# ebeauce/Seismic_BPMF

Measured on AMD Instinct MI355X. Metric: million network-CC-samples/s (matched filter), higher is better.
Workload: dtype f32

## Files before the change

### seismic_bpmf_amd/csrc/mf_split.h

```cpp
#pragma once
#include <hip/hip_runtime.h>
#include <cstdint>

namespace bpmf {
namespace sp {

typedef _Float16 f16x8 __attribute__((ext_vector_type(8)));
typedef float f32x16 __attribute__((ext_vector_type(16)));
typedef float f32x4 __attribute__((ext_vector_type(4)));
typedef float f32x4u __attribute__((ext_vector_type(4), aligned(4)));
typedef int i32x4 __attribute__((ext_vector_type(4)));
typedef int i32x2 __attribute__((ext_vector_type(2)));
typedef unsigned u32x4 __attribute__((ext_vector_type(4)));

constexpr int NT = 2;
constexpr int LAGS_W = 1024 * NT;
constexpr int WAVES = 4;
constexpr int THREADS = 64 * WAVES;
constexpr int LAGS_WG = WAVES * LAGS_W;
constexpr int W_LOADS = 10;
constexpr int W_CHUNKS = 64 * W_LOADS;
constexpr int W_BYTES = (W_CHUNKS + W_CHUNKS / 8) * 16;
constexpr int B_LOADS = 4;
constexpr int BAND_BYTES = 64 * B_LOADS * 16;
constexpr int BAND_PLANE = BAND_BYTES / 2;
constexpr int WAVE_LDS = W_BYTES + BAND_BYTES;
constexpr int WG_LDS = WAVES * WAVE_LDS;
constexpr int MAX_KS = 26;
constexpr int BAND_LEAD = 40;
constexpr int S_TARGET = 14;
constexpr int S_CLAMP = 60;
constexpr float SP_MAX_NORM = 1000.0f;

__host__ __device__ inline int nks_of(int L) { return (L + 38 + 15) / 16; }
__host__ __device__ inline int max_segment_len() { return (16 * MAX_KS - 38) / 8 * 8; }
__host__ __device__ inline int n_segments_of(int L) { return (L + max_segment_len() - 1) / max_segment_len(); }
__host__ __device__ inline int segment_len_of(int L)
{
    const int n = n_segments_of(L);
    return ((L + n - 1) / n + 7) / 8 * 8;
}
__host__ __device__ inline int max_template_len() { return 4096; }
__host__ __device__ inline int band_e_dwords(int nks) { return 8 * nks + 32; }
__host__ __device__ inline int band_o_off(int nks)
{
    const int e = band_e_dwords(nks);
    return e + ((17 - e % 32) + 32) % 32;
}
__host__ __device__ inline size_t split_row_bytes(size_t N) { return ((N + 7) / 8) * 32; }

__host__ __device__ inline int scale_exp_of(unsigned maxbits)
{
    if (maxbits == 0u || maxbits >= 0x7f800000u) return 0;
    const int e = (int)(maxbits >> 23) - 127;
    int s = S_TARGET - e;
    if (s > S_CLAMP) s = S_CLAMP;
    if (s < -S_CLAMP) s = -S_CLAMP;
    return s;
}
__host__ __device__ inline float pow2f(int s)
{
    union { unsigned u; float f; } v;
    v.u = (unsigned)(s + 127) << 23;
    return v.f;
}

constexpr float LO_SCALE = 2048.0f;

__device__ __forceinline__ void split_one(float v, float lo_scale, unsigned short& hi, unsigned short& lo)
{
    const _Float16 h = (_Float16)v;
    const float res = v - (float)h;
    const _Float16 l = (_Float16)(res * lo_scale);
    hi = __builtin_bit_cast(unsigned short, h);
    lo = __builtin_bit_cast(unsigned short, l);
}

__global__ __launch_bounds__(256) void sp_absmax_kernel(const float* __restrict__ data, size_t N,
                                                        unsigned* __restrict__ maxbits)
{
    const float* d = data + (size_t)blockIdx.y * N;
    unsigned m = 0;
    for (size_t i = (size_t)blockIdx.x * 256 + threadIdx.x; i < N; i += (size_t)gridDim.x * 256)
        m = max(m, __float_as_uint(d[i]) & 0x7fffffffu);
#pragma unroll
    for (int o = 32; o > 0; o >>= 1) m = max(m, (unsigned)__shfl_xor((int)m, o));
    if ((threadIdx.x & 63) == 0 && m) atomicMax(maxbits + blockIdx.y, m);
}

__global__ void sp_scale_kernel(const unsigned* __restrict__ maxbits, int n_ch, int* __restrict__ s_exp,
                                float* __restrict__ scd)
{
    const int ch = blockIdx.x * blockDim.x + threadIdx.x;
    if (ch >= n_ch) return;
    const int s = scale_exp_of(maxbits[ch]);
    s_exp[ch] = s;
    scd[ch] = pow2f(-s);
}

__global__ __launch_bounds__(256) void sp_split_data_kernel(const float* __restrict__ data, size_t N, size_t NQ,
                                                            const int* __restrict__ s_exp, u32x4* __restrict__ out)
{
    const size_t q = (size_t)blockIdx.x * 256 + threadIdx.x;
    if (q >= NQ) return;
    const size_t ch = blockIdx.y;
    const float* d = data + ch * N + 8 * q;
    const float sc = pow2f(s_exp[ch]);
    float v[8];
    if (8 * q + 8 <= N) {
        const f32x4u a = *(const f32x4u*)d, b = *(const f32x4u*)(d + 4);
#pragma unroll
        for (int i = 0; i < 4; ++i) { v[i] = a[i]; v[4 + i] = b[i]; }
    } else {
#pragma unroll
        for (int i = 0; i < 8; ++i) v[i] = 8 * q + i < N ? d[i] : 0.0f;
    }
    unsigned short hi[8], lo[8];
#pragma unroll
    for (int i = 0; i < 8; ++i) split_one(v[i] * sc, LO_SCALE, hi[i], lo[i]);
    u32x4 oh, ol;
#pragma unroll
    for (int i = 0; i < 4; ++i) {
        oh[i] = (unsigned)hi[2 * i] | ((unsigned)hi[2 * i + 1] << 16);
        ol[i] = (unsigned)lo[2 * i] | ((unsigned)lo[2 * i + 1] << 16);
    }
    u32x4* o = out + (ch * NQ + q) * 2;
    o[0] = oh;
    o[1] = ol;
}

__global__ __launch_bounds__(64) void sp_band_kernel(const float* __restrict__ tmpl, const int* __restrict__ mv,
                                                     int L, int n_seg, int seg_len, unsigned* __restrict__ bands,
                                                     float* __restrict__ sct)
{
    const size_t tc = blockIdx.x / (unsigned)n_seg;
    const int seg = (int)(blockIdx.x % (unsigned)n_seg);
    const int lane = threadIdx.x;
    const float* x = tmpl + tc * (size_t)L;
    unsigned m = 0;
    for (int l = lane; l < L; l += 64) m = max(m, __float_as_uint(x[l]) & 0x7fffffffu);
#pragma unroll
    for (int o = 32; o > 0; o >>= 1) m = max(m, (unsigned)__shfl_xor((int)m, o));
    const int s = scale_exp_of(m);
    const float sc = pow2f(s);
    if (lane == 0 && seg == 0) sct[tc] = pow2f(-s);
    const int mvc = mv[tc];
    const int r = ((mvc % 8) + 8) % 8;
    const int nks = nks_of(seg_len);
    const int e_d = band_e_dwords(nks), o_off = band_o_off(nks);
    unsigned* img = bands + (size_t)blockIdx.x * (BAND_BYTES / 4);
    auto elem = [&](int i, int p) -> unsigned {
        const int ls = i - BAND_LEAD - r;
        const int l = seg * seg_len + ls;
        if (ls < 0 || ls >= seg_len || l >= L) return 0u;
        unsigned short hi, lo;
        split_one(x[l] * sc, 1.0f, hi, lo);
        return p ? lo : hi;
    };
    for (int w = lane; w < BAND_BYTES / 4; w += 64) {
        const int p = w >= BAND_PLANE / 4 ? 1 : 0;
        const int n = w - p * (BAND_PLANE / 4);
        unsigned val = 0u;
        if (n < e_d) val = elem(2 * n, p) | (elem(2 * n + 1, p) << 16);
        else if (n >= o_off && n < o_off + e_d) {
            const int k = n - o_off;
            val = elem(2 * k + 1, p) | (elem(2 * k + 2, p) << 16);
        }
        img[w] = val;
    }
}

__device__ __forceinline__ bool sp_tile_of_block(unsigned bid, int T, int n_lag_blocks, int& t, long long& lag_block)
{
    const unsigned xcd = bid & 7u, i = bid >> 3;
    const unsigned total = (unsigned)n_lag_blocks * (unsigned)T;
    const unsigned per_xcd = (total + 7u) >> 3;
    const unsigned flat = xcd * per_xcd + i;
    t = (int)(flat % (unsigned)T);
    lag_block = (long long)(flat / (unsigned)T);
    return i < per_xcd && flat < total;
}

#define SP_SB __builtin_amdgcn_sched_barrier(0)
#define SP_RD2(dst, addr, o0) \
    asm volatile("ds_read2_b32 %0, %1 offset0:%2 offset1:%3" : "=v"(dst) : "v"(addr), "n"(o0), "n"((o0) + 1))
#define SP_RD128(dst, addr, off) asm volatile("ds_read_b128 %0, %1 offset:%2" : "=v"(dst) : "v"(addr), "n"(off))

struct Frags {
    i32x2 a[2][2];
    i32x4 b[NT][2];
};

__device__ __forceinline__ f16x8 sp_h8(i32x2 lo, i32x2 hi)
{
    const i32x4 v = {lo[0], lo[1], hi[0], hi[1]};
    return __builtin_bit_cast(f16x8, v);
}
__device__ __forceinline__ f16x8 sp_h8(i32x4 v) { return __builtin_bit_cast(f16x8, v); }

template <bool NETWORK_SUM, bool STEP1, int ABLATE = 0, bool SEGMENTED = false>
__global__ __launch_bounds__(THREADS, 2) void mf_split_kernel(
    const u32x4* __restrict__ sdata, const unsigned* __restrict__ bands, const float* __restrict__ sct,
    const float* __restrict__ scd, const int4* __restrict__ chan_rec, const float* __restrict__ e_d,
    const int2* __restrict__ range, int L, long long N, int T, int n_ch, long long n_corr, int step,
    float* __restrict__ out, int n_lag_blocks, int lag_block0, int prio, int n_seg, int seg_len)
{
    extern __shared__ __attribute__((aligned(16))) char sp_smem[];
    const int tid = threadIdx.x;
    const int lane = tid & 63;
    const int wv = __builtin_amdgcn_readfirstlane(tid >> 6);
    const int a = lane & 31;
    const int g = lane >> 5;
    const int nks = nks_of(seg_len);
    const bool kprio = (((blockIdx.x >> 3) ^ (blockIdx.x >> 8)) & 1u) != 0;

    int t;
    long long lag_block;
    if (!sp_tile_of_block(blockIdx.x, T, n_lag_blocks, t, lag_block)) return;
    lag_block += lag_block0;
    const int2 rgi = range[t];
    const long long lag0 = lag_block * LAGS_WG + (long long)wv * LAGS_W;
    const int2 rg = make_int2(rgi.x * step, rgi.y * step);
    const long long nwin = N - L + 1;
    const size_t row_bytes = split_row_bytes((size_t)N);

    f32x16 sum[NT];
#pragma unroll
    for (int u = 0; u < NT; ++u)
#pragma unroll
        for (int r = 0; r < 16; ++r) sum[u][r] = 0.0f;

    const bool wave_valid = rg.x <= rg.y && !(lag0 > rg.y || lag0 + LAGS_W - 1 < rg.x);
    const bool wave_inside = lag0 >= rg.x && lag0 + LAGS_W - 1 <= rg.y;
    const long long lag_w = lag0 + 32 * a + 4 * g;

    if (wave_valid) {
        char* wbase = sp_smem + wv * WAVE_LDS;
        char* bbase = wbase + W_BYTES;
        const unsigned w_st = (unsigned)(size_t)wbase + 16u * (unsigned)(lane + (lane >> 3));
        const unsigned b_st = (unsigned)(size_t)bbase + 16u * (unsigned)lane;
        const unsigned b_rd = (unsigned)(size_t)wbase + 144u * (unsigned)a + 32u * (unsigned)g;
        const int odd = a & 1;
        const int a_dw = 4 * g - ((a + 1) >> 1) + BAND_LEAD / 2 + (odd ? band_o_off(nks) : 0);
        const unsigned a_rd = (unsigned)(size_t)bbase + 4u * (unsigned)a_dw;
        const int4* __restrict__ recs = chan_rec + (size_t)t * (n_ch + 2);

        u32x4 rd[W_LOADS], rt[B_LOADS];
        auto issue_stage = [&](int ch, int mvc, int sg) {
            const __amdgpu_buffer_rsrc_t rs = __builtin_amdgcn_make_buffer_rsrc(
                (void*)((const char*)sdata + (size_t)ch * row_bytes), 0, (int)row_bytes, 0x00020000);
            const long long q0 = (lag0 >> 3) + (long long)(mvc >> 3) + (long long)sg * (seg_len >> 3);
            const unsigned o = (unsigned)(q0 * 32 + 16 * lane);
            if (q0 >= 0) {
#pragma unroll
                for (int i = 0; i < W_LOADS; ++i)
                    rd[i] = __builtin_bit_cast(u32x4, __builtin_amdgcn_raw_buffer_load_b128(rs, (int)(o + 1024u * i), 0, 0));
            } else {
                unsigned oo = o;
#pragma unroll
                for (int i = 0; i < W_LOADS; ++i) {
                    asm volatile("" : "+v"(oo));
                    rd[i] = __builtin_bit_cast(u32x4, __builtin_amdgcn_raw_buffer_load_b128(rs, (int)oo, 0, 0));
                    oo += 1024u;
                }
            }
            const u32x4* bi = (const u32x4*)(bands + (((size_t)t * n_ch + ch) * n_seg + sg) * (BAND_BYTES / 4)) + lane;
#pragma unroll
            for (int i = 0; i < B_LOADS; ++i) rt[i] = bi[64 * i];
        };
        auto write_stage = [&]() {
#pragma unroll
            for (int i = 0; i < B_LOADS; ++i)
                asm volatile("ds_write_b128 %0, %1 offset:%2" :: "v"(b_st), "v"(rt[i]), "n"(1024 * i) : "memory");
#pragma unroll
            for (int i = 0; i < W_LOADS; ++i)
                asm volatile("ds_write_b128 %0, %1 offset:%2" :: "v"(w_st), "v"(rd[i]), "n"(1152 * i) : "memory");
        };

        int4 rec = recs[0];
        int4 rec1 = recs[1];
        int ri = 0, seg = 0;
        f32x16 acc[NT];
        f32x4 ed[NT][4];
        if (ABLATE < 2 && rec.x >= 0) issue_stage(rec.x, rec.y, 0);
        while (rec.x >= 0) {
            const int ch = rec.x;
            const bool last_seg = !SEGMENTED || seg == n_seg - 1;
            if constexpr (ABLATE < 2) write_stage();
            const float w = __int_as_float(rec.z);
            const int mvc = rec.y;
            const float rt_n = __int_as_float(rec.w);
            const float s_t = sct[(size_t)t * n_ch + ch];
            const float s_d = scd[ch];
            const float s_td = s_t * s_d;
            const int4 rec2 = recs[ri + 2];
            const float* edc = e_d + (size_t)ch * (size_t)nwin;
            if (!last_seg) {
            } else if constexpr (ABLATE >= 1) {
#pragma unroll
                for (int u = 0; u < NT; ++u)
#pragma unroll
                    for (int i = 0; i < 4; ++i) ed[u][i] = (f32x4){1.0f, 1.0f, 1.0f, 1.0f};
            } else if (wave_inside) {
#pragma unroll
                for (int u = 0; u < NT; ++u)
#pragma unroll
                    for (int i = 0; i < 4; ++i) ed[u][i] = *(const f32x4u*)(edc + lag_w + 1024 * u + 8 * i + mvc);
            } else {
#pragma unroll
                for (int u = 0; u < NT; ++u)
#pragma unroll
                    for (int i = 0; i < 4; ++i) {
                        const long long lag = lag_w + 1024 * u + 8 * i;
                        if (lag + 3 >= rg.x && lag <= rg.y) ed[u][i] = *(const f32x4u*)(edc + lag + mvc);
                        else ed[u][i] = (f32x4){0.0f, 0.0f, 0.0f, 0.0f};
                    }
            }
            if constexpr (ABLATE < 2) {
                if (!last_seg) issue_stage(rec.x, rec.y, seg + 1);
                else if (rec1.x >= 0) issue_stage(rec1.x, rec1.y, 0);
            }

            if (!SEGMENTED || seg == 0) {
#pragma unroll
                for (int u = 0; u < NT; ++u)
#pragma unroll
                    for (int r = 0; r < 16; ++r) acc[u][r] = 0.0f;
            }

            unsigned ap = a_rd, ap2 = a_rd + BAND_PLANE, bp = b_rd;
            Frags f[2];
#define SP_REQ(s, dw, off)                                                    \
    SP_RD2(f[s].a[0][0], ap, (dw));     SP_RD2(f[s].a[0][1], ap, (dw) + 2);   \
    SP_RD128(f[s].b[0][0], bp, (off));         SP_RD128(f[s].b[1][0], bp, (off) + 4608);      \
    SP_RD128(f[s].b[0][1], bp, (off) + 16);    SP_RD128(f[s].b[1][1], bp, (off) + 4608 + 16); \
    SP_RD2(f[s].a[1][0], ap2, (dw));    SP_RD2(f[s].a[1][1], ap2, (dw) + 2)
#define SP_MFMA(acc, av, bv) acc = __builtin_amdgcn_mfma_f32_32x32x16_f16(av, bv, acc, 0, 0, 0)
#define SP_WAIT(n) asm volatile("s_waitcnt lgkmcnt(%0)" :: "n"(n) : "memory")
#define SP_STEP(cur, nxt, dw, off)                                                          \
    {                                                                                        \
        SP_WAIT(5); SP_SB;                                                                   \
        const f16x8 ah = sp_h8(f[cur].a[0][0], f[cur].a[0][1]);                              \
        const f16x8 hs = ah * (_Float16)(1.0f / LO_SCALE);       \
        SP_MFMA(acc[0], ah, sp_h8(f[cur].b[0][0]));                                          \
        SP_SB;                                                                               \
        SP_RD2(f[nxt].a[0][0], ap, (dw)); SP_RD2(f[nxt].a[0][1], ap, (dw) + 2);              \
        SP_WAIT(6); SP_SB;                                                                   \
        SP_MFMA(acc[1], ah, sp_h8(f[cur].b[1][0]));                                          \
        SP_SB;                                                                               \
        SP_RD128(f[nxt].b[0][0], bp, (off)); SP_RD128(f[nxt].b[1][0], bp, (off) + 4608);     \
        SP_WAIT(7); SP_SB;                                                                   \
        SP_MFMA(acc[0], hs, sp_h8(f[cur].b[0][1]));                                          \
        SP_SB;                                                                               \
        SP_RD128(f[nxt].b[0][1], bp, (off) + 16); SP_RD128(f[nxt].b[1][1], bp, (off) + 4608 + 16); \
        SP_WAIT(8); SP_SB;                                                                   \
        SP_MFMA(acc[1], hs, sp_h8(f[cur].b[1][1]));                                          \
        SP_SB;                                                                               \
        SP_RD2(f[nxt].a[1][0], ap2, (dw)); SP_RD2(f[nxt].a[1][1], ap2, (dw) + 2);            \
        SP_WAIT(8); SP_SB;                                                                   \
        const f16x8 al = sp_h8(f[cur].a[1][0], f[cur].a[1][1]);                              \
        SP_MFMA(acc[0], al, sp_h8(f[cur].b[0][0]));                                          \
        SP_SB;                                                                               \
        SP_MFMA(acc[1], al, sp_h8(f[cur].b[1][0]));                                          \
        SP_SB;                                                                               \
    }
#define SP_STEP_LAST(cur)                                                                    \
    {                                                                                        \
        SP_WAIT(5); SP_SB;                                                                   \
        const f16x8 ah = sp_h8(f[cur].a[0][0], f[cur].a[0][1]);                              \
        const f16x8 hs = ah * (_Float16)(1.0f / LO_SCALE);                                   \
        SP_MFMA(acc[0], ah, sp_h8(f[cur].b[0][0]));                                          \
        SP_WAIT(4); SP_SB;                                                                   \
        SP_MFMA(acc[1], ah, sp_h8(f[cur].b[1][0]));                                          \
        SP_WAIT(3); SP_SB;                                                                   \
        SP_MFMA(acc[0], hs, sp_h8(f[cur].b[0][1]));                                          \
        SP_WAIT(2); SP_SB;                                                                   \
        SP_MFMA(acc[1], hs, sp_h8(f[cur].b[1][1]));                                          \
        SP_WAIT(0); SP_SB;                                                                   \
        const f16x8 al = sp_h8(f[cur].a[1][0], f[cur].a[1][1]);                              \
        SP_MFMA(acc[0], al, sp_h8(f[cur].b[0][0]));                                          \
        SP_SB;                                                                               \
        SP_MFMA(acc[1], al, sp_h8(f[cur].b[1][0]));                                          \
        SP_SB;                                                                               \
    }
            SP_SB;
            if (prio & 1) __builtin_amdgcn_s_setprio(0);
            if ((prio & 2) && kprio) __builtin_amdgcn_s_setprio(2);
            SP_REQ(0, 0, 0);
            const int npair = nks >> 1;
            for (int p = 0; p < npair; ++p) {
                SP_STEP(0, 1, 8, 64);
                SP_STEP(1, 0, 16, 144);
                ap += 64;
                ap2 += 64;
                bp += 144;
            }
            if (nks & 1) { SP_STEP_LAST(0); }
            asm volatile("s_waitcnt lgkmcnt(0)" ::: "memory");
            SP_SB;
            if (prio & 1) __builtin_amdgcn_s_setprio(1);
            else if (prio & 2) __builtin_amdgcn_s_setprio(0);
#undef SP_REQ
#undef SP_WAIT
#undef SP_MFMA
#undef SP_STEP
#undef SP_STEP_LAST

            if (!last_seg) {
                ++seg;
                continue;
            }
            seg = 0;
#pragma unroll
            for (int u = 0; u < NT; ++u) {
#pragma unroll
                for (int r = 0; r < 16; ++r) {
                    const float num = acc[u][r] * s_td;
                    const float nrm = rt_n * ed[u][r >> 2][r & 3];
                    float cc;
                    if (prio & 4)
                        cc = nrm > 1.0e-6f ? num / sqrtf(nrm) : 0.0f;
                    else
                        cc = nrm < SP_MAX_NORM ? num * nrm : 0.0f;
                    if (NETWORK_SUM && STEP1 && wave_inside) {
                        sum[u][r] = __fmaf_rn(w, cc, sum[u][r]);
                    } else {
                        const long long lag = lag_w + 1024 * u + 8 * (r >> 2) + (r & 3);
                        const bool ok = lag >= rg.x && lag <= rg.y && (STEP1 || (unsigned)lag % (unsigned)step == 0);
                        if (!ok) cc = 0.0f;
                        if (!NETWORK_SUM) {
                            if (ok)
                                out[((size_t)t * n_corr + (STEP1 ? lag : (long long)((unsigned)lag / (unsigned)step))) * n_ch + ch] = cc;
                        } else {
                            sum[u][r] = __fmaf_rn(w, cc, sum[u][r]);
                        }
                    }
                }
            }
            rec = rec1;
            rec1 = rec2;
            ++ri;
        }
    }
    if (NETWORK_SUM) {
#pragma unroll
        for (int u = 0; u < NT; ++u) {
#pragma unroll
            for (int i = 0; i < 4; ++i) {
                const long long lag = lag_w + 1024 * u + 8 * i;
                float* dst = out + (size_t)t * n_corr + lag;
// ... 19 lines not shown
```

### seismic_bpmf_amd/csrc/mf_split.hip

```cpp
#include "mf_split.h"
#include "mf_split_api.h"
#include <algorithm>

namespace bpmf {
namespace sp {

namespace {
struct DayRegion { u32x4* planes; unsigned* maxbits; int* s_exp; float* scd; };
DayRegion carve_day(void* base, size_t N, size_t n_ch)
{
    char* p = (char*)base;
    DayRegion r;
    size_t o = 0;
    r.planes = (u32x4*)(p + o);  o += align_up(n_ch * split_row_bytes(N), 256);
    r.maxbits = (unsigned*)(p + o); o += align_up(n_ch * sizeof(unsigned), 256);
    r.s_exp = (int*)(p + o);     o += align_up(n_ch * sizeof(int), 256);
    r.scd = (float*)(p + o);
    return r;
}
}

size_t day_region_bytes(size_t N, size_t n_ch)
{
    return align_up(n_ch * split_row_bytes(N), 256) + 3 * align_up(n_ch * 4, 256);
}

size_t batch_region_bytes(size_t T, size_t n_ch, size_t L)
{
    const size_t n_seg = L ? (size_t)n_segments_of((int)std::min<size_t>(L, (size_t)max_template_len())) : 1;
    return align_up(T * n_ch * n_seg * (size_t)BAND_BYTES, 256) + align_up(T * n_ch * sizeof(float), 256);
}

bool usable(size_t L, size_t N)
{
    return L <= (size_t)max_template_len() && N < ((size_t)1 << 30) - 8192;
}

int prepare_day(const float* d_data, size_t N, size_t n_ch, void* day_region, hipStream_t stream)
{
    const DayRegion r = carve_day(day_region, N, n_ch);
    const size_t NQ = (N + 7) / 8;
    if (n_ch > 65535) {
        set_error("mf.split16: more than 65535 channels");
        return -1;
    }
    BPMF_HIP_CHECK(hipMemsetAsync(r.maxbits, 0, n_ch * sizeof(unsigned), stream));
    const unsigned nb = (unsigned)std::min<size_t>(256, (N + 4095) / 4096);
    sp_absmax_kernel<<<dim3(nb, (unsigned)n_ch), dim3(256), 0, stream>>>(d_data, N, r.maxbits);
    BPMF_LAUNCH_CHECK();
    sp_scale_kernel<<<dim3((unsigned)((n_ch + 63) / 64)), dim3(64), 0, stream>>>(r.maxbits, (int)n_ch, r.s_exp, r.scd);
    BPMF_LAUNCH_CHECK();
    sp_split_data_kernel<<<dim3((unsigned)((NQ + 255) / 256), (unsigned)n_ch), dim3(256), 0, stream>>>(d_data, N, NQ, r.s_exp,
                                                                                                     r.planes);
    BPMF_LAUNCH_CHECK();
    return 0;
}

int run(const float* d_templates, const int32_t* d_moveouts, const void* day_region, void* batch_region,
        const int4* chan_rec, const float* e_d, const int2* range, size_t step, size_t L, size_t N, size_t T,
        size_t n_ch, size_t n_corr, int network_sum, int sqrt_norm, size_t nb_lo, size_t nb_cnt, float* d_cc_out,
        hipStream_t stream)
{
    const DayRegion r = carve_day(const_cast<void*>(day_region), N, n_ch);
    const int n_seg = n_segments_of((int)L), seg_len = segment_len_of((int)L);
    unsigned* bands = (unsigned*)batch_region;
    float* sct = (float*)((char*)batch_region + align_up(T * n_ch * (size_t)n_seg * (size_t)BAND_BYTES, 256));
    if (T * n_ch * (size_t)n_seg >= 0x7fffffffull || T * (nb_cnt + 8) >= 0x7fffffffull) {
        set_error("mf.split16: grid too large");
        return -1;
    }
    sp_band_kernel<<<dim3((unsigned)(T * n_ch * (size_t)n_seg)), dim3(64), 0, stream>>>(d_templates, d_moveouts, (int)L, n_seg,
                                                                                      seg_len, bands, sct);
    BPMF_LAUNCH_CHECK();
    const dim3 grid((unsigned)(8 * ((T * nb_cnt + 7) / 8)));
#define BPMF_SP_LAUNCH(NS, S1)                                                                                       \
    do { if (n_seg > 1) BPMF_SP_LAUNCH2(NS, S1, true); else BPMF_SP_LAUNCH2(NS, S1, false); } while (0)
#define BPMF_SP_LAUNCH2(NS, S1, SG)                                                                                  \
    do {                                                                                                             \
        auto kfn = mf_split_kernel<NS, S1, 0, SG>;                                                                   \
                                             \
        kfn<<<grid, dim3(THREADS), WG_LDS, stream>>>(r.planes, bands, sct, r.scd, chan_rec, e_d, range, (int)L,      \
                                                     (long long)N, (int)T, (int)n_ch, (long long)n_corr, (int)step,   \
                                                     d_cc_out, (int)nb_cnt, (int)nb_lo, sqrt_norm ? 4 : 0, n_seg,     \
                                                     seg_len);                                                        \
    } while (0)
    if (network_sum && step == 1) BPMF_SP_LAUNCH(true, true);
    else if (network_sum) BPMF_SP_LAUNCH(true, false);
    else if (step == 1) BPMF_SP_LAUNCH(false, true);
    else BPMF_SP_LAUNCH(false, false);
#undef BPMF_SP_LAUNCH
#undef BPMF_SP_LAUNCH2
    BPMF_LAUNCH_CHECK();
    return 0;
}

}
}
```

### seismic_bpmf_amd/csrc/mf.hip

```cpp
#include "common.h"
#include "host_call.h"
#include "mf_split_api.h"
#include "mf_full_api.h"
#include <system_error>
#include <thread>
#include <chrono>
#include <vector>
#include <mutex>
#include <utility>
#include <cstring>
#include <algorithm>
#include "../../include/bpmf_hip.h"

#include <cstdlib>

namespace bpmf {

typedef float f32x16 __attribute__((ext_vector_type(16)));


__device__ __forceinline__ int2 mf_lag_range(bool any, long long mv_min, long long mv_max, long long step,
                                             long long L, long long N, long long n_corr, int exclusive_last)
{
    int2 r = make_int2(1, 0);
// ... 126 lines not shown
            for (size_t i = 0; i < len; ++i) {
                const double v = (double)s_in[i];
                acc = acc + v * v;
                s_out[i] = acc;
            }
        }
        __syncthreads();
        for (size_t i = lane; i < len; i += 64) lo[n0 + i] = s_out[i];
        __syncthreads();
    }
}

__global__ void mf_csum_offsets_kernel(const double* __restrict__ tot, size_t n_ch, size_t nq,
                                       double* __restrict__ off, size_t q_lo, size_t q_hi)
{
    size_t ch = (size_t)blockIdx.x * blockDim.x + threadIdx.x;
    if (ch >= n_ch) return;
    const double* tr = tot + ch * nq;
    double* orow = off + ch * nq;
    double acc = q_lo ? orow[q_lo - 1] + tr[q_lo - 1] : 0.0;
    size_t q = q_lo;
    for (; q + 16 <= q_hi; q += 16) {
        double v[16];
#pragma unroll
        for (int i = 0; i < 16; ++i) v[i] = tr[q + i];
#pragma unroll
        for (int i = 0; i < 16; ++i) {
            orow[q + i] = acc;
            acc = acc + v[i];
        }
    }
    for (; q < q_hi; ++q) {
        orow[q] = acc;
        acc = acc + tr[q];
    }
}

__global__ void mf_window_energy_kernel(const double* __restrict__ local,
                                        const double* __restrict__ off, size_t n_ch, size_t N,
                                        size_t nq, size_t L, size_t nwin, int sqrt_norm,
                                        float* __restrict__ e_d, size_t w_lo, size_t w_hi)
{
    size_t j = w_lo + (size_t)blockIdx.x * blockDim.x + threadIdx.x;
    size_t ch = blockIdx.y;
    if (j >= w_hi) return;
    const double* lo = local + ch * N;
    const double* of = off + ch * nq;
    size_t nh = j + L - 1;
    double hi = of[nh / CSUM_CHUNK] + lo[nh];
    double low = 0.0;
    if (j > 0) low = of[(j - 1) / CSUM_CHUNK] + lo[j - 1];
    const float e = (float)(hi - low);
    e_d[ch * nwin + j] = sqrt_norm ? e : 1.0f / sqrtf(e);
}


template <bool SQRT_NORM>
__device__ __forceinline__ float mf_cc_of(float num, float nt, float nd)
{
    if constexpr (SQRT_NORM) {
        const float den2 = nt * nd;
        return den2 > 1.0e-6f ? num / sqrtf(den2) : 0.0f;
    } else {
        const float nrm = nt * nd;
        return nrm < MAX_NORM ? num * nrm : 0.0f;
    }
}

constexpr int MF_THREADS = 256;
constexpr int MF_LAGS_PER_WAVE = 1024;
constexpr int MF_LAGS_PER_WG = 4096;
constexpr int MF_REC_TERMINATORS = 12;

typedef float f32x4 __attribute__((ext_vector_type(4)));
typedef float f32x4u __attribute__((ext_vector_type(4), aligned(4)));

__device__ __forceinline__ int mf_pad(int x) { return x + (x >> 4); }

__host__ __device__ inline int mf_kpad(int L) { return (L + 15 + 15) / 16 * 16; }
__host__ __device__ inline int mf_band_len(int L) { return mf_kpad(L) + 16; }
__host__ __device__ inline int mf_window_len(int L) { return MF_LAGS_PER_WG - 16 + mf_kpad(L); }
__host__ __device__ inline int mf_buf_floats(int L)
{
    const int W = mf_window_len(L);
    return mf_band_len(L) + (W + (W >> 4) + 1);
}
__host__ inline size_t mf_lds_bytes(int L) { return ((size_t)2 * mf_buf_floats(L) + 64) * sizeof(float); }

__device__ __forceinline__ bool mf_tile_of_block(unsigned bid, int T, int n_lag_blocks, int& t,
                                                 long long& lag_block)
{
    const unsigned xcd = bid & 7u, i = bid >> 3;
    const unsigned total = (unsigned)n_lag_blocks * (unsigned)T;
    const unsigned per_xcd = (total + 7u) >> 3;
    const unsigned flat = xcd * per_xcd + i;
    t = (int)(flat % (unsigned)T);
    lag_block = (long long)(flat / (unsigned)T);
    return i < per_xcd && flat < total;
}

template <int NR, int STRIDE>
__device__ __forceinline__ void mf_stage_rows(float (&rd)[NR], __amdgpu_buffer_rsrc_t rs,
                                              long long first, int idx)
{
    const unsigned o = (unsigned)((first + idx) * 4);
    if (first >= 0) {
// ... 886 lines not shown
    if (option(OPT_MF_WAVE_KERNEL) == 0 || mf_kpad((int)L) > 272) {
        v.family = MF_WORKGROUP;
        v.maxr = need_r <= 20 && need_t <= 5 ? 20 : 24;
        v.maxt = v.maxr == 20 ? 5 : 9;
        v.lags_wg = MF_LAGS_PER_WG;
        v.lds = mf_lds_bytes((int)L);
        v.grid = mf_grid(T, n_lag_blocks);
        return v;
    }
    v.family = MF_WAVE;
    const size_t waves4 = T * n_lag_blocks * 4;
    v.ntile = waves4 >= 8192 ? 4 : (waves4 >= 1024 ? 2 : 1);
    const long forced = option(OPT_MF_TILES_PER_WAVE);
    if (forced == 1 || forced == 2 || forced == 4) v.ntile = (int)forced;
    v.maxr = mf_wave_maxr(v.ntile);
    v.maxt = MF_WAVE_MAXT;
    v.fused = v.ntile < 4 && n_ch <= 256 && option(OPT_MF_FUSED_PROLOGUE) != 0;
    v.prologue = !v.fused;
    const long csplit_max = option(OPT_MF_CHANNEL_SPLIT);
    v.csplit = v.ntile == 1 && v.fused && network_sum && v.step1 && n_ch <= 32 && !ranged && csplit_max > 0 &&
               waves4 * 4 <= (size_t)csplit_max;
    v.lags_wg = v.csplit ? (size_t)256 : (size_t)4 * 256 * v.ntile;
    const size_t n_blocks_w = (n_offsets + v.lags_wg - 1) / v.lags_wg;
    if (T * (n_blocks_w + 8) >= 0x7fffffffull) v.refusal = MF_GRID_TOO_LARGE;
    v.grid = mf_grid(T, n_blocks_w);
    const int Wbuf = v.ntile < 4 ? 64 * v.maxr : 256 * v.ntile - 16 + mf_kpad((int)L);
    v.lds = (size_t)4 * (mf_band_len((int)L) + (Wbuf + 2 * (Wbuf >> 4) + 2 + 63) / 64 * 64 + 64) * sizeof(float) + 256 +
            (v.fused ? 64 + (n_ch + MF_REC_TERMINATORS) * sizeof(int4) : 0) +
            (v.csplit ? n_ch * 256 * sizeof(float) : 0);
    return v;
}

}

using namespace bpmf;

extern "C" size_t bpmf_mf_workspace_bytes(size_t L, size_t N, size_t T, size_t S, size_t C)
{
    return mf_carve(nullptr, L, N, T, S * C).bytes;
}

extern "C" size_t bpmf_mf_full_workspace_bytes(size_t L, size_t N, size_t T, size_t S, size_t C)
{
    return mf_carve_full(nullptr, L, N, T, S * C).ws.bytes;
}

static int mf_prepare_range(const float* d_data, size_t L, size_t N, size_t n_ch, const MfWorkspace& ws,
                            hipStream_t stream, size_t samp_lo, size_t samp_hi)
{
    const size_t nq = (N + CSUM_CHUNK - 1) / CSUM_CHUNK;
    const size_t nwin = N - L + 1;
    const size_t q_lo = samp_lo / CSUM_CHUNK, q_hi = (samp_hi + CSUM_CHUNK - 1) / CSUM_CHUNK;
    if (q_hi <= q_lo) return 0;
    {
        size_t n = n_ch * (q_hi - q_lo);
        mf_csum_local_kernel<<<dim3((unsigned)((n + 63) / 64)), dim3(64), 0, stream>>>(
            d_data, n_ch, N, nq, ws.local, ws.tot, q_lo, q_hi - q_lo);
        BPMF_LAUNCH_CHECK();
    }
    mf_csum_offsets_kernel<<<dim3((unsigned)((n_ch + 63) / 64)), dim3(64), 0, stream>>>(
        ws.tot, n_ch, nq, ws.off, q_lo, q_hi);
    BPMF_LAUNCH_CHECK();
    const size_t w_lo = samp_lo >= L - 1 ? samp_lo - (L - 1) : 0;
    const size_t w_hi = samp_hi >= N ? nwin : (samp_hi >= L - 1 ? std::min(nwin, samp_hi - (L - 1)) : 0);
    if (w_hi > w_lo) {
        mf_window_energy_kernel<<<dim3((unsigned)((w_hi - w_lo + 255) / 256), (unsigned)n_ch), dim3(256), 0,
                                  stream>>>(ws.local, ws.off, n_ch, N, nq, L, nwin,
                                            option(OPT_MF_COMPAT_SQRT_NORM) != 0 ? 1 : 0, ws.e_d, w_lo, w_hi);
        BPMF_LAUNCH_CHECK();
    }
    return 0;
}

extern "C" int bpmf_mf_prepare_data_dev(const float* d_data, size_t L, size_t N, size_t S, size_t C,
                                        void* d_workspace, size_t workspace_bytes,
                                        bpmf_stream_t stream_)
{
    hipStream_t stream = (hipStream_t)stream_;
    const size_t n_ch = S * C;
    if (!d_data || !d_workspace || N < L || L == 0 || n_ch == 0) {
        set_error("bpmf_mf_prepare_data_dev: bad argument");
        return -1;
    }
    MfWorkspace ws = mf_carve(d_workspace, L, N, 0, n_ch);
    if (workspace_bytes < ws.bytes) {
        set_error("bpmf_mf_prepare_data_dev: workspace too small (%zu < %zu)", workspace_bytes,
                  ws.bytes);
        return -1;
    }
    if (option(OPT_MF_COMPAT_SEQUENTIAL_CSUM) != 0) {
        const size_t nq = (N + CSUM_CHUNK - 1) / CSUM_CHUNK;
        const size_t nwin = N - L + 1;
        mf_csum_sequential_kernel<<<dim3((unsigned)n_ch), dim3(64), 0, stream>>>(d_data, N, nq, ws.local, ws.off);
        BPMF_LAUNCH_CHECK();
        mf_window_energy_kernel<<<dim3((unsigned)((nwin + 255) / 256), (unsigned)n_ch), dim3(256), 0,
                                  stream>>>(ws.local, ws.off, n_ch, N, nq, L, nwin,
                                            option(OPT_MF_COMPAT_SQRT_NORM) != 0 ? 1 : 0, ws.e_d, 0, nwin);
        BPMF_LAUNCH_CHECK();
    } else if (int rc = mf_prepare_range(d_data, L, N, n_ch, ws, stream, 0, N)) {
        return rc;
    }
    const bool with_split = ws.sp_day && sp::usable(L, N);
    split_day_note(d_workspace, d_data, N, n_ch, with_split);
    full_day_note(d_workspace, d_data, N, n_ch, false);
    if (with_split) return sp::prepare_day(d_data, N, n_ch, ws.sp_day, stream);
    return 0;
}

extern "C" int bpmf_mf_prepare_data_full_dev(const float* d_data, size_t L, size_t N, size_t S, size_t C,
                                             void* d_workspace, size_t workspace_bytes, bpmf_stream_t stream_)
{
    hipStream_t stream = (hipStream_t)stream_;
    const size_t n_ch = S * C;
    if (!d_data || !d_workspace || N < L || L == 0 || n_ch == 0 || N > 0x7fffffffull) {
        set_error("bpmf_mf_prepare_data_full_dev: bad argument");
        return -1;
    }
// ... 389 lines not shown
```

Before: 4453.

## Split data into separate hi/lo planes with guard padding and 2-sample alignment

Result: no change. 4457 (median of 3 runs) (+0.1%).

```diff
diff --git a/seismic_bpmf_amd/csrc/mf_split.h b/seismic_bpmf_amd/csrc/mf_split.h
--- a/seismic_bpmf_amd/csrc/mf_split.h
+++ b/seismic_bpmf_amd/csrc/mf_split.h
@@ -19,7 +19,9 @@
 constexpr int THREADS = 64 * WAVES;
 constexpr int LAGS_WG = WAVES * LAGS_W;
 constexpr int W_LOADS = 10;
+constexpr int P_LOADS = W_LOADS / 2;
 constexpr int W_CHUNKS = 64 * W_LOADS;
+constexpr int W_SAMPLES = 8 * 64 * P_LOADS;
 constexpr int W_BYTES = (W_CHUNKS + W_CHUNKS / 8) * 16;
 constexpr int B_LOADS = 4;
 constexpr int BAND_BYTES = 64 * B_LOADS * 16;
@@ -28,11 +30,13 @@
 constexpr int WG_LDS = WAVES * WAVE_LDS;
 constexpr int MAX_KS = 26;
 constexpr int BAND_LEAD = 40;
+constexpr int GUARD = W_SAMPLES + 128;
 constexpr int S_TARGET = 14;
 constexpr int S_CLAMP = 60;
 constexpr float SP_MAX_NORM = 1000.0f;
 
 __host__ __device__ inline int nks_of(int L) { return (L + 38 + 15) / 16; }
+__host__ __device__ inline int nks_run_of(int L) { return (L + 32 + 15) / 16; }
 __host__ __device__ inline int max_segment_len() { return (16 * MAX_KS - 38) / 8 * 8; }
 __host__ __device__ inline int n_segments_of(int L) { return (L + max_segment_len() - 1) / max_segment_len(); }
 __host__ __device__ inline int segment_len_of(int L)
@@ -47,7 +51,9 @@
     const int e = band_e_dwords(nks);
     return e + ((17 - e % 32) + 32) % 32;
 }
-__host__ __device__ inline size_t split_row_bytes(size_t N) { return ((N + 7) / 8) * 32; }
+__host__ __device__ inline size_t split_plane_chunks(size_t N) { return (N + 7) / 8 + 2 * (size_t)(GUARD / 8); }
+__host__ __device__ inline size_t split_plane_bytes(size_t N) { return split_plane_chunks(N) * 16; }
+__host__ __device__ inline size_t split_row_bytes(size_t N) { return 2 * split_plane_bytes(N); }
 
 __host__ __device__ inline int scale_exp_of(unsigned maxbits)
 {
@@ -101,9 +107,17 @@
 __global__ __launch_bounds__(256) void sp_split_data_kernel(const float* __restrict__ data, size_t N, size_t NQ,
                                                             const int* __restrict__ s_exp, u32x4* __restrict__ out)
 {
-    const size_t q = (size_t)blockIdx.x * 256 + threadIdx.x;
-    if (q >= NQ) return;
+    const size_t j = (size_t)blockIdx.x * 256 + threadIdx.x;
+    const size_t PC = NQ + 2 * (size_t)(GUARD / 8);
+    if (j >= PC) return;
     const size_t ch = blockIdx.y;
+    u32x4* o = out + ch * 2 * PC + j;
+    if (j < (size_t)(GUARD / 8) || j >= NQ + (size_t)(GUARD / 8)) {
+        o[0] = (u32x4){0u, 0u, 0u, 0u};
+        o[PC] = (u32x4){0u, 0u, 0u, 0u};
+        return;
+    }
+    const size_t q = j - (size_t)(GUARD / 8);
     const float* d = data + ch * N + 8 * q;
     const float sc = pow2f(s_exp[ch]);
     float v[8];
@@ -124,9 +138,8 @@
         oh[i] = (unsigned)hi[2 * i] | ((unsigned)hi[2 * i + 1] << 16);
         ol[i] = (unsigned)lo[2 * i] | ((unsigned)lo[2 * i + 1] << 16);
     }
-    u32x4* o = out + (ch * NQ + q) * 2;
     o[0] = oh;
-    o[1] = ol;
+    o[PC] = ol;
 }
 
 __global__ __launch_bounds__(64) void sp_band_kernel(const float* __restrict__ tmpl, const int* __restrict__ mv,
@@ -145,7 +158,7 @@
     const float sc = pow2f(s);
     if (lane == 0 && seg == 0) sct[tc] = pow2f(-s);
     const int mvc = mv[tc];
-    const int r = ((mvc % 8) + 8) % 8;
+    const int r = mvc & 1;
     const int nks = nks_of(seg_len);
     const int e_d = band_e_dwords(nks), o_off = band_o_off(nks);
     unsigned* img = bands + (size_t)blockIdx.x * (BAND_BYTES / 4);
@@ -212,6 +225,7 @@
     const int a = lane & 31;
     const int g = lane >> 5;
     const int nks = nks_of(seg_len);
+    const int nks_run = nks_run_of(seg_len);
     const bool kprio = (((blockIdx.x >> 3) ^ (blockIdx.x >> 8)) & 1u) != 0;
 
     int t;
@@ -222,7 +236,7 @@
     const long long lag0 = lag_block * LAGS_WG + (long long)wv * LAGS_W;
     const int2 rg = make_int2(rgi.x * step, rgi.y * step);
     const long long nwin = N - L + 1;
-    const size_t row_bytes = split_row_bytes((size_t)N);
+    const size_t plane_bytes = split_plane_bytes((size_t)N);
 
     f32x16 sum[NT];
 #pragma unroll
@@ -237,7 +251,7 @@
     if (wave_valid) {
         char* wbase = sp_smem + wv * WAVE_LDS;
         char* bbase = wbase + W_BYTES;
-        const unsigned w_st = (unsigned)(size_t)wbase + 16u * (unsigned)(lane + (lane >> 3));
+        const unsigned w_st = (unsigned)(size_t)wbase + 16u * (unsigned)(2 * lane + (lane >> 2));
         const unsigned b_st = (unsigned)(size_t)bbase + 16u * (unsigned)lane;
         const unsigned b_rd = (unsigned)(size_t)wbase + 144u * (unsigned)a + 32u * (unsigned)g;
         const int odd = a & 1;
@@ -247,20 +261,25 @@
 
         u32x4 rd[W_LOADS], rt[B_LOADS];
         auto issue_stage = [&](int ch, int mvc, int sg) {
-            const __amdgpu_buffer_rsrc_t rs = __builtin_amdgcn_make_buffer_rsrc(
-                (void*)((const char*)sdata + (size_t)ch * row_bytes), 0, (int)row_bytes, 0x00020000);
-            const long long q0 = (lag0 >> 3) + (long long)(mvc >> 3) + (long long)sg * (seg_len >> 3);
-            const unsigned o = (unsigned)(q0 * 32 + 16 * lane);
-            if (q0 >= 0) {
-#pragma unroll
-                for (int i = 0; i < W_LOADS; ++i)
-                    rd[i] = __builtin_bit_cast(u32x4, __builtin_amdgcn_raw_buffer_load_b128(rs, (int)(o + 1024u * i), 0, 0));
+            const char* row = (const char*)sdata + (size_t)ch * (2 * plane_bytes);
+            const __amdgpu_buffer_rsrc_t rs_h = __builtin_amdgcn_make_buffer_rsrc((void*)row, 0, (int)plane_bytes, 0x00020000);
+            const __amdgpu_buffer_rsrc_t rs_l =
+                __builtin_amdgcn_make_buffer_rsrc((void*)(row + plane_bytes), 0, (int)plane_bytes, 0x00020000);
+            const long long x0 = (long long)GUARD + lag0 + (long long)(mvc & ~1) + (long long)sg * seg_len;
+            const unsigned o = (unsigned)(x0 * 2 + 16 * lane);
+            if (x0 >= 0) {
+#pragma unroll
+                for (int i = 0; i < P_LOADS; ++i) {
+                    rd[2 * i] = __builtin_bit_cast(u32x4, __builtin_amdgcn_raw_buffer_load_b128(rs_h, (int)(o + 1024u * i), 0, 0));
+                    rd[2 * i + 1] = __builtin_bit_cast(u32x4, __builtin_amdgcn_raw_buffer_load_b128(rs_l, (int)(o + 1024u * i), 0, 0));
+                }
             } else {
                 unsigned oo = o;
 #pragma unroll
-                for (int i = 0; i < W_LOADS; ++i) {
+                for (int i = 0; i < P_LOADS; ++i) {
                     asm volatile("" : "+v"(oo));
-                    rd[i] = __builtin_bit_cast(u32x4, __builtin_amdgcn_raw_buffer_load_b128(rs, (int)oo, 0, 0));
+                    rd[2 * i] = __builtin_bit_cast(u32x4, __builtin_amdgcn_raw_buffer_load_b128(rs_h, (int)oo, 0, 0));
+                    rd[2 * i + 1] = __builtin_bit_cast(u32x4, __builtin_amdgcn_raw_buffer_load_b128(rs_l, (int)oo, 0, 0));
                     oo += 1024u;
                 }
             }
@@ -274,7 +293,7 @@
                 asm volatile("ds_write_b128 %0, %1 offset:%2" :: "v"(b_st), "v"(rt[i]), "n"(1024 * i) : "memory");
 #pragma unroll
             for (int i = 0; i < W_LOADS; ++i)
-                asm volatile("ds_write_b128 %0, %1 offset:%2" :: "v"(w_st), "v"(rd[i]), "n"(1152 * i) : "memory");
+                asm volatile("ds_write_b128 %0, %1 offset:%2" :: "v"(w_st), "v"(rd[i]), "n"(2304 * (i >> 1) + 16 * (i & 1)) : "memory");
         };
 
         int4 rec = recs[0];
@@ -301,20 +320,15 @@
                 for (int u = 0; u < NT; ++u)
 #pragma unroll
                     for (int i = 0; i < 4; ++i) ed[u][i] = (f32x4){1.0f, 1.0f, 1.0f, 1.0f};
-            } else if (wave_inside) {
+            } else {
+                const __amdgpu_buffer_rsrc_t rn =
+                    __builtin_amdgcn_make_buffer_rsrc((void*)(edc - 4), 0, (int)((nwin + 8) * 4), 0x00020000);
+                const unsigned no = (unsigned)((lag_w + mvc + 4) * 4);
 #pragma unroll
                 for (int u = 0; u < NT; ++u)
 #pragma unroll
-                    for (int i = 0; i < 4; ++i) ed[u][i] = *(const f32x4u*)(edc + lag_w + 1024 * u + 8 * i + mvc);
-            } else {
-#pragma unroll
-                for (int u = 0; u < NT; ++u)
-#pragma unroll
-                    for (int i = 0; i < 4; ++i) {
-                        const long long lag = lag_w + 1024 * u + 8 * i;
-                        if (lag + 3 >= rg.x && lag <= rg.y) ed[u][i] = *(const f32x4u*)(edc + lag + mvc);
-                        else ed[u][i] = (f32x4){0.0f, 0.0f, 0.0f, 0.0f};
-                    }
+                    for (int i = 0; i < 4; ++i)
+                        ed[u][i] = __builtin_bit_cast(f32x4, __builtin_amdgcn_raw_buffer_load_b128(rn, (int)(no + 4096u * u + 32u * i), 0, 0));
             }
             if constexpr (ABLATE < 2) {
                 if (!last_seg) issue_stage(rec.x, rec.y, seg + 1);
@@ -387,7 +401,7 @@
             if (prio & 1) __builtin_amdgcn_s_setprio(0);
             if ((prio & 2) && kprio) __builtin_amdgcn_s_setprio(2);
             SP_REQ(0, 0, 0);
-            const int npair = nks >> 1;
+            const int npair = nks_run >> 1;
             for (int p = 0; p < npair; ++p) {
                 SP_STEP(0, 1, 8, 64);
                 SP_STEP(1, 0, 16, 144);
@@ -395,7 +409,7 @@
                 ap2 += 64;
                 bp += 144;
             }
-            if (nks & 1) { SP_STEP_LAST(0); }
+            if (nks_run & 1) { SP_STEP_LAST(0); }
             asm volatile("s_waitcnt lgkmcnt(0)" ::: "memory");
             SP_SB;
             if (prio & 1) __builtin_amdgcn_s_setprio(1);
diff --git a/seismic_bpmf_amd/csrc/mf_split.hip b/seismic_bpmf_amd/csrc/mf_split.hip
--- a/seismic_bpmf_amd/csrc/mf_split.hip
+++ b/seismic_bpmf_amd/csrc/mf_split.hip
@@ -50,8 +50,8 @@
     BPMF_LAUNCH_CHECK();
     sp_scale_kernel<<<dim3((unsigned)((n_ch + 63) / 64)), dim3(64), 0, stream>>>(r.maxbits, (int)n_ch, r.s_exp, r.scd);
     BPMF_LAUNCH_CHECK();
-    sp_split_data_kernel<<<dim3((unsigned)((NQ + 255) / 256), (unsigned)n_ch), dim3(256), 0, stream>>>(d_data, N, NQ, r.s_exp,
-                                                                                                     r.planes);
+    sp_split_data_kernel<<<dim3((unsigned)((split_plane_chunks(N) + 255) / 256), (unsigned)n_ch), dim3(256), 0, stream>>>(
+        d_data, N, NQ, r.s_exp, r.planes);
     BPMF_LAUNCH_CHECK();
     return 0;
 }
```

## Restructure matched-filter data-norm prefix sums with LDS-staged totals and windowed norms

Applied to the files above, without the earlier changes.

New measurement: 4426 before, 4439 after, median of 6. About the same (+0.3%).

```diff
diff --git a/seismic_bpmf_amd/csrc/mf.hip b/seismic_bpmf_amd/csrc/mf.hip
--- a/seismic_bpmf_amd/csrc/mf.hip
+++ b/seismic_bpmf_amd/csrc/mf.hip
@@ -202,6 +202,236 @@
     if (j > 0) low = of[(j - 1) / CSUM_CHUNK] + lo[j - 1];
     const float e = (float)(hi - low);
     e_d[ch * nwin + j] = sqrt_norm ? e : 1.0f / sqrtf(e);
+}
+
+
+typedef float f32x4a __attribute__((ext_vector_type(4), aligned(4)));
+typedef float f32x4v __attribute__((ext_vector_type(4)));
+typedef double f64x2v __attribute__((ext_vector_type(2)));
+
+constexpr int TOT_PIECE = 64;
+constexpr int TOT_ROW = TOT_PIECE + 4;
+
+template <bool FULL>
+__device__ __forceinline__ double mf_totals_chain(const float* __restrict__ data, float* s_x, const size_t* s_base,
+                                                  const int* s_len, int lane, double* __restrict__ ck, int n_ck)
+{
+    double acc = 0.0;
+    const int sub = lane >> 4, col = (lane & 15) * 4;
+    f32x4v v[16];
+    auto fetch = [&](int r) {
+        const int p = r * TOT_PIECE + col;
+#pragma unroll
+        for (int k = 0; k < 16; ++k) {
+            const int m = 4 * k + sub;
+            const float* g = data + s_base[m] + p;
+            if constexpr (FULL) {
+                v[k] = *(const f32x4a*)g;
+            } else {
+                const int len = s_len[m];
+                v[k][0] = p + 0 < len ? g[0] : 0.0f;
+                v[k][1] = p + 1 < len ? g[1] : 0.0f;
+                v[k][2] = p + 2 < len ? g[2] : 0.0f;
+                v[k][3] = p + 3 < len ? g[3] : 0.0f;
+            }
+        }
+    };
+    fetch(0);
+    for (int r = 0; r < CSUM_CHUNK / TOT_PIECE; ++r) {
+#pragma unroll
+        for (int k = 0; k < 16; ++k) *(f32x4v*)&s_x[(4 * k + sub) * TOT_ROW + col] = v[k];
+        __syncthreads();
+        if (r + 1 < CSUM_CHUNK / TOT_PIECE) fetch(r + 1);
+        if (r < n_ck) ck[r] = acc;
+#pragma unroll
+        for (int i = 0; i < TOT_PIECE / 4; ++i) {
+            const f32x4v w = *(const f32x4v*)&s_x[lane * TOT_ROW + 4 * i];
+            double x = (double)w[0]; acc = acc + x * x;
+            x = (double)w[1]; acc = acc + x * x;
+            x = (double)w[2]; acc = acc + x * x;
+            x = (double)w[3]; acc = acc + x * x;
+        }
+        __syncthreads();
+    }
+    return acc;
+}
+
+__global__ __launch_bounds__(64) void mf_csum_totals_kernel(const float* __restrict__ data, size_t n_ch, size_t N,
+                                                            size_t nq, double* __restrict__ tot,
+                                                            double* __restrict__ front, size_t q_lo, size_t q_cnt)
+{
+    __shared__ float s_x[64 * TOT_ROW];
+    __shared__ size_t s_base[64];
+    __shared__ int s_len[64];
+    const int lane = threadIdx.x;
+    const size_t n_items = n_ch * q_cnt;
+    size_t idx = (size_t)blockIdx.x * 64 + lane;
+    const bool mine = idx < n_items;
+    if (!mine) idx = n_items - 1;
+    const size_t ch = idx / q_cnt, q = q_lo + idx % q_cnt;
+    const size_t n0 = q * CSUM_CHUNK;
+    const int len = (int)(n0 + CSUM_CHUNK < N ? (size_t)CSUM_CHUNK : N - n0);
+    s_base[lane] = ch * N + n0;
+    s_len[lane] = len;
+    __syncthreads();
+    double* ck = front + ch * ((N + TOT_PIECE - 1) / TOT_PIECE) + n0 / TOT_PIECE;
+    const int n_ck = mine ? (len + TOT_PIECE - 1) / TOT_PIECE : 0;
+    const double acc = __all(len == CSUM_CHUNK) ? mf_totals_chain<true>(data, s_x, s_base, s_len, lane, ck, n_ck)
+                                                : mf_totals_chain<false>(data, s_x, s_base, s_len, lane, ck, n_ck);
+    if (mine) tot[ch * nq + q] = acc;
+}
+
+template <bool INCLUSIVE>
+__device__ __forceinline__ double mf_lds_chain(double* s, int n, double acc)
+{
+    f64x2v x[4][4];
+    auto rd = [&](f64x2v (&r)[4], int i) {
+        i = std::min(i, n - 8);
+#pragma unroll
+        for (int k = 0; k < 4; ++k) r[k] = *(const f64x2v*)&s[i + 2 * k];
+    };
+    rd(x[0], 0);
+    rd(x[1], 8);
+    rd(x[2], 16);
+    for (int i = 0; i < n; i += 32) {
+#pragma unroll
+        for (int u = 0; u < 4; ++u) {
+#pragma unroll
+            for (int k = 0; k < 4; ++k) {
+#pragma unroll
+                for (int e = 0; e < 2; ++e) {
+                    const double t = x[u][k][e];
+                    if (INCLUSIVE) {
+                        acc = acc + t;
+                        x[u][k][e] = acc;
+                    } else {
+                        x[u][k][e] = acc;
+                        acc = acc + t;
+                    }
+                }
+            }
+#pragma unroll
+            for (int k = 0; k < 4; ++k) *(f64x2v*)&s[i + 8 * u + 2 * k] = x[u][k];
+            rd(x[(u + 3) & 3], i + 8 * u + 24);
+        }
+    }
+    return acc;
+}
+
+__global__ __launch_bounds__(64) void mf_csum_offsets_wave_kernel(const double* __restrict__ tot, size_t nq,
+                                                                  double* __restrict__ off, size_t q_lo, size_t q_hi)
+{
+    __shared__ double s_t[CSUM_CHUNK];
+    constexpr int B = CSUM_CHUNK, PER = B / 64;
+    const int lane = threadIdx.x;
+    const double* tr = tot + (size_t)blockIdx.x * nq;
+    double* orow = off + (size_t)blockIdx.x * nq;
+    double acc = q_lo ? orow[q_lo - 1] + tr[q_lo - 1] : 0.0;
+    double cur[PER];
+#pragma unroll
+    for (int k = 0; k < PER; ++k) cur[k] = tr[std::min(q_lo + (size_t)(k * 64 + lane), q_hi - 1)];
+    for (size_t q0 = q_lo; q0 < q_hi; q0 += B) {
+        const int cnt = (int)std::min<size_t>(B, q_hi - q0);
+#pragma unroll
+        for (int k = 0; k < PER; ++k) s_t[k * 64 + lane] = cur[k];
+        __syncthreads();
+        double nxt[PER] = {};
+        if (q0 + B < q_hi) {
+#pragma unroll
+            for (int k = 0; k < PER; ++k) nxt[k] = tr[std::min(q0 + B + (size_t)(k * 64 + lane), q_hi - 1)];
+        }
+        if (lane == 0) acc = mf_lds_chain<false>(s_t, (cnt + 31) & ~31, acc);
+        __syncthreads();
+#pragma unroll
+        for (int k = 0; k < PER; ++k)
+            if (k * 64 + lane < cnt) orow[q0 + k * 64 + lane] = s_t[k * 64 + lane];
+        __syncthreads();
+#pragma unroll
+        for (int k = 0; k < PER; ++k) cur[k] = nxt[k];
+    }
+}
+
+constexpr int NRM_SPAN = 4 * CSUM_CHUNK;
+constexpr int NRM_THREADS = 256;
+constexpr int NRM_PAD = 2;
+constexpr int NRM_MAX_CHUNKS = 8;
+constexpr size_t NRM_MAX_L = (NRM_MAX_CHUNKS - 1) * CSUM_CHUNK - NRM_SPAN;
+
+static size_t mf_norms_lds_bytes(size_t L)
+{
+    const size_t n = align_up(NRM_SPAN + L - 1, TOT_PIECE);
+    return (NRM_MAX_CHUNKS + n + NRM_PAD * (n / TOT_PIECE)) * sizeof(double);
+}
+
+__global__ __launch_bounds__(NRM_THREADS) void mf_window_norms_kernel(const float* __restrict__ data,
+                                                                      const double* __restrict__ off,
+                                                                      const double* __restrict__ front, size_t N,
+                                                                      size_t nq, size_t L, size_t nwin,
+                                                                      float* __restrict__ e_d, size_t w_lo, size_t w_hi)
+{
+    extern __shared__ double nrm_lds[];
+    double* s_off = nrm_lds;
+    double* s_lo = nrm_lds + NRM_MAX_CHUNKS;
+    const int tid = threadIdx.x;
+    const size_t ch = blockIdx.y;
+    const size_t s0 = (w_lo / NRM_SPAN + blockIdx.x) * NRM_SPAN;
+    const size_t j0 = std::max(w_lo, s0), j1 = std::min(w_hi, s0 + NRM_SPAN);
+    const size_t base = j0 / TOT_PIECE * TOT_PIECE, qa = base / CSUM_CHUNK;
+    const int cnt = (int)(j1 + L - 1 - base);
+    const int cntp = (cnt + TOT_PIECE - 1) & ~(TOT_PIECE - 1);
+    const int npiece = cntp / TOT_PIECE;
+    const int nchunk = (int)((base + cnt - 1) / CSUM_CHUNK - qa) + 1;
+    const float* d = data + ch * N + base;
+    const double* fr = front + ch * ((N + TOT_PIECE - 1) / TOT_PIECE) + base / TOT_PIECE;
+    auto slot = [](int i) { return i + NRM_PAD * (i / TOT_PIECE); };
+
+    double acc0 = 0.0;
+    if (tid < npiece) acc0 = fr[tid];
+    if (tid < nchunk) s_off[tid] = off[ch * nq + qa + tid];
+    const int nquad = cnt >> 2;
+    for (int qb = tid; qb < nquad; qb += 4 * NRM_THREADS) {
+        f32x4v v[4];
+#pragma unroll
+        for (int k = 0; k < 4; ++k) v[k] = *(const f32x4a*)(d + 4 * std::min(qb + k * NRM_THREADS, nquad - 1));
+#pragma unroll
+        for (int k = 0; k < 4; ++k) {
+            const int i = 4 * (qb + k * NRM_THREADS);
+            if (i + 4 > cnt) break;
+            f64x2v a, b;
+            double x = (double)v[k][0]; a[0] = x * x;
+            x = (double)v[k][1]; a[1] = x * x;
+            x = (double)v[k][2]; b[0] = x * x;
+            x = (double)v[k][3]; b[1] = x * x;
+            *(f64x2v*)&s_lo[slot(i)] = a;
+            *(f64x2v*)&s_lo[slot(i) + 2] = b;
+        }
+    }
+    {
+        const int i = (cnt & ~3) + tid;
+        if (i < cntp) {
+            double x = 0.0;
+            if (i < cnt) x = (double)d[i];
+            s_lo[slot(i)] = x * x;
+        }
+    }
+    __syncthreads();
+    if (tid < npiece) mf_lds_chain<true>(s_lo + tid * (TOT_PIECE + NRM_PAD), TOT_PIECE, acc0);
+    __syncthreads();
+    float* e_row = e_d + ch * nwin;
+    for (size_t j = j0 + tid; j < j1; j += NRM_THREADS) {
+        const size_t nh = j + L - 1;
+        const double hi = s_off[nh / CSUM_CHUNK - qa] + s_lo[slot((int)(nh - base))];
+        double low = 0.0;
+        if (j % CSUM_CHUNK == 0) {
+            if (j > 0) low = s_off[j / CSUM_CHUNK - qa];
+        } else if (j == base) {
+            low = s_off[0] + fr[0];
+        } else {
+            low = s_off[(j - 1) / CSUM_CHUNK - qa] + s_lo[slot((int)(j - 1 - base))];
+        }
+        const float e = (float)(hi - low);
+        e_row[j] = 1.0f / sqrtf(e);
+    }
 }
 
 
@@ -1194,6 +1424,23 @@
     const size_t nwin = N - L + 1;
     const size_t q_lo = samp_lo / CSUM_CHUNK, q_hi = (samp_hi + CSUM_CHUNK - 1) / CSUM_CHUNK;
     if (q_hi <= q_lo) return 0;
+    const size_t w_lo = samp_lo >= L - 1 ? samp_lo - (L - 1) : 0;
+    const size_t w_hi = samp_hi >= N ? nwin : (samp_hi >= L - 1 ? std::min(nwin, samp_hi - (L - 1)) : 0);
+    if (option(OPT_MF_COMPAT_SQRT_NORM) == 0 && L <= NRM_MAX_L) {
+        const size_t n = n_ch * (q_hi - q_lo);
+        mf_csum_totals_kernel<<<dim3((unsigned)((n + 63) / 64)), dim3(64), 0, stream>>>(d_data, n_ch, N, nq, ws.tot, ws.local,
+                                                                                        q_lo, q_hi - q_lo);
+        BPMF_LAUNCH_CHECK();
+        mf_csum_offsets_wave_kernel<<<dim3((unsigned)n_ch), dim3(64), 0, stream>>>(ws.tot, nq, ws.off, q_lo, q_hi);
+        BPMF_LAUNCH_CHECK();
+        if (w_hi > w_lo) {
+            const size_t n_span = (w_hi - 1) / NRM_SPAN - w_lo / NRM_SPAN + 1;
+            mf_window_norms_kernel<<<dim3((unsigned)n_span, (unsigned)n_ch), dim3(NRM_THREADS), mf_norms_lds_bytes(L),
+                                     stream>>>(d_data, ws.off, ws.local, N, nq, L, nwin, ws.e_d, w_lo, w_hi);
+            BPMF_LAUNCH_CHECK();
+        }
+        return 0;
+    }
     {
         size_t n = n_ch * (q_hi - q_lo);
         mf_csum_local_kernel<<<dim3((unsigned)((n + 63) / 64)), dim3(64), 0, stream>>>(
@@ -1203,8 +1450,6 @@
     mf_csum_offsets_kernel<<<dim3((unsigned)((n_ch + 63) / 64)), dim3(64), 0, stream>>>(
         ws.tot, n_ch, nq, ws.off, q_lo, q_hi);
     BPMF_LAUNCH_CHECK();
-    const size_t w_lo = samp_lo >= L - 1 ? samp_lo - (L - 1) : 0;
-    const size_t w_hi = samp_hi >= N ? nwin : (samp_hi >= L - 1 ? std::min(nwin, samp_hi - (L - 1)) : 0);
     if (w_hi > w_lo) {
         mf_window_energy_kernel<<<dim3((unsigned)((w_hi - w_lo + 255) / 256), (unsigned)n_ch), dim3(256), 0,
                                   stream>>>(ws.local, ws.off, n_ch, N, nq, L, nwin,
```
